# facebookresearch/vggsfm

Hardware: AMD Instinct MI355X
Metric: BA LM-iterations/sec (higher is better)
Workload: dtype f64

## Files before the change

vggsfm_amd/ba.py:

```python
import copy
import ctypes
from dataclasses import dataclass
from typing import Optional

import math
import os

import numpy as np
import torch

from . import _lib
from .ba_options import LOSS_ID, TERMINATION, BundleAdjustmentOptions

MODEL_ID = {"SIMPLE_PINHOLE": 0, "SIMPLE_RADIAL": 1}
GROUP = 16
CHUNK = 1024
SUB = 32
MIN_CHUNK = 128
OVERLAP_FACTORIZATION = False
OVERLAP_MIN_OBS, OVERLAP_MIN_FRAMES = 1_000_000, 8 * GROUP
TILE_BATCHES = 3
CHOL_CUS = 32


# ... 629 lines not shown
    overlap = OVERLAP_FACTORIZATION if overlap is None else bool(overlap)
    nb = TILE_BATCHES if (overlap and int(obs_cam.shape[0]) >= OVERLAP_MIN_OBS and S >= OVERLAP_MIN_FRAMES) else 1
    merged = nb == 1 and int(obs_cam.shape[0]) < MERGED_TILE_MAX_OBS
    merged_slots = slots[0] if merged else None
    chunk_desc, entries, tile_desc, obs_slot, nseg, batch_desc = build_schur_tiles(
        row_ptr, obs_cam, max_chunks=slots, num_batches=nb, later_scale=(cus - CHOL_CUS) / cus,
        merged_slots=merged_slots, block_rows=block_rows, simple=int(obs_cam.shape[0]) < SIMPLE_WORKLIST_MAX_OBS, num_cams=S)
    prob = DeviceProblem(cam_q, cam_t, intr, pts, row_ptr, obs_cam, obs_uv, col_ptr, cobs_pt, cobs_uv, chunk_desc,
                         entries, tile_desc, obs_slot, nseg, MODEL_ID[camera_type], cam_const=cam_const,
                         batch_desc=batch_desc, chol_split=chol_split, cam_perm=cam_perm, merged_tile_launch=merged,
                         refine_focal=bool(refine_focal_length), refine_extra=bool(refine_extra_params))
    if first_group is not None:
        kd_max = 2 if camera_type == "SIMPLE_RADIAL" else 1
        prob.chol_first_blk = envelope_blocks(first_group, S, 6 * S + kd_max * n_intr).to(dev)
    return prob, valid_idx, deleted


def window_bundle_adjustment(points3d, extrinsics, intrinsics, tracks, masks, num_existing_points, extra_params=None,
                             shared_camera=True, camera_type="SIMPLE_RADIAL", options=None):
    options = copy.deepcopy(options) if options is not None else BundleAdjustmentOptions()
    options.refine_focal_length = False
    options.refine_extra_params = False
    valid = masks.bool().sum(0) >= 2
    order = torch.cumsum(valid.long(), 0) - 1
    constant = valid & (order < num_existing_points)
    return bundle_adjustment(points3d, extrinsics, intrinsics, tracks, masks, None, extra_params, shared_camera,
                             camera_type, options, False, constant_points=constant, constant_pose_frames=[0],
                             filter_negative_depth=False)


def _c_options(options: BundleAdjustmentOptions, overlap=True):
    so = options.solver_options
    return _lib.BAOptions(so.max_num_iterations, so.max_num_consecutive_invalid_steps, int(so.jacobi_scaling),
                          so.function_tolerance, so.gradient_tolerance, so.parameter_tolerance,
                          so.initial_trust_region_radius, so.max_trust_region_radius, so.min_trust_region_radius,
                          so.min_lm_diagonal, so.max_lm_diagonal, so.min_relative_decrease,
                          CHOL_CUS if (overlap and OVERLAP_FACTORIZATION) else 0)


def _summary_dict(summ, log, n):
    its = [dict(iteration=l.iteration, cost=l.cost, cost_change=l.cost_change, gradient_max_norm=l.gradient_max_norm,
                step_norm=l.step_norm, relative_decrease=l.relative_decrease, radius=l.radius,
                successful=bool(l.successful)) for l in log[:n]]
    return dict(initial_cost=summ.initial_cost, final_cost=summ.final_cost, num_iterations=summ.num_iterations,
                num_successful_steps=summ.num_successful_steps, num_unsuccessful_steps=summ.num_unsuccessful_steps,
                termination=summ.termination, termination_str=TERMINATION.get(summ.termination, "?"),
                n_reduced=summ.n_reduced, iterations=its)


def apply_launch_hooks(L):
    glue = _hook("VGGSFM_LEGACY_GLUE")
    if glue is not None:
        L.vgg_ba_set_tile_rhs(2 | (4 if glue == "1" else 0))


def solve(problem: DeviceProblem, options: Optional[BundleAdjustmentOptions] = None, workspace=None):
    L = _lib.lib()
    apply_launch_hooks(L)
    options = options or BundleAdjustmentOptions()
    problem.refine_focal = options.refine_focal_length
    problem.refine_extra = options.refine_extra_params
    problem.loss = LOSS_ID[options.loss_function_type]
    problem.loss_scale = options.loss_function_scale
    cp = problem.c_struct()
    co = _c_options(options)
    nbytes = L.vgg_ba_workspace_bytes(ctypes.byref(cp), ctypes.byref(co))
    if workspace is None or workspace.numel() < nbytes:
        workspace = torch.empty(nbytes, dtype=torch.uint8, device=problem.pts.device)
    summ = _lib.BASummary()
    cap = options.solver_options.max_num_iterations + 2
    log = (_lib.BAIteration * cap)()
    _lib.check(L.vgg_ba_solve(ctypes.byref(cp), ctypes.byref(co), workspace, workspace.numel(), ctypes.byref(summ), log, cap,
                              _lib.stream_ptr()), "vgg_ba_solve")
    out = _summary_dict(summ, log, summ.num_log)
    if options.print_summary:
        print(f"Bundle adjustment report: residuals {problem.num_obs * 2}, parameters reduced {summ.n_reduced}, "
              f"iterations {summ.num_iterations}, cost {summ.initial_cost:.6g} -> {summ.final_cost:.6g}, "
              f"{out['termination_str']}")
    return out, workspace


POSE_COMPONENTS = ("rx", "ry", "rz", "tx", "ty", "tz")


@dataclass
class BACovariance:
    pose: Optional[torch.Tensor]
    intrinsics: Optional[torch.Tensor]
    pose_intrinsics: Optional[torch.Tensor]
    points: Optional[torch.Tensor]
    reduced: Optional[torch.Tensor]
    columns: list
    num_active: int
    variance_factor: float
    cost: float


def covariance_columns(problem: DeviceProblem):
    C, NI = problem.cam_t.shape[0], problem.intr.shape[0]
    names = [nm for nm, on in (("f", problem.refine_focal), ("k", problem.refine_extra and problem.camera_model == 1)) if on]
    frame = list(range(C)) if problem.cam_perm is None else [int(f) for f in problem.cam_perm.tolist()]
    cols = [("pose", frame[c], comp) for c in range(C) for comp in POSE_COMPONENTS]
    cols += [("intrinsics", 0 if NI == 1 else frame[a], nm) for a in range(NI) for nm in names]
    return cols


# ... 175 lines not shown
```

vggsfm_amd/csrc/ba.hip:

```cpp
#include <mutex>
#include <vector>

#include "ba_types.hpp"

namespace vgg {

Tuning g_tuning = {0, -1, 0, 0, 2, 0};
Profiler g_prof;

__global__ void init_kernel(DevProblem pb, Ws w, vgg_ba_options opt, int rank, int world) {
  const Dims& d = pb.d;
  const int j = blockIdx.x * blockDim.x + threadIdx.x;
  if (j == 0) {
    Ctl c;
    memset(&c, 0, sizeof(c));
    c.radius = opt.initial_trust_region_radius; c.decrease_factor = 2.0; c.need_lin = 1; c.rank = rank; c.world = world;
    *w.ctl = c;
    w.gmax_pts[0] = 0; for (int i = 0; i < 4; ++i) w.stepsum[i] = 0;
  }
  if (j < d.n_red) {
    bool act;
    if (j < 6 * d.C) {
      const int c = j / 6, k = j - 6 * c;
      const unsigned f = pb.cam_const ? pb.cam_const[c] : 0u;
      act = (pb.col_ptr[c + 1] > pb.col_ptr[c]) || world > 1;
      if (f & 1u) act = false;
      if (k >= 3 && (f & (2u << (k - 3)))) act = false;
    } else {
      const int a = (j - 6 * d.C) / d.kd;
      act = !(pb.intr_const && pb.intr_const[a]);
      if (!d.shared && world == 1 && !(pb.col_ptr[a + 1] > pb.col_ptr[a])) act = false;
    }
    w.active[j] = act ? 1 : 0;
    w.scale_c[j] = 1.0;
  }
}

__device__ __forceinline__ void begin_iteration(const Ws& w, const vgg_ba_options& opt) {
  Ctl* c = w.ctl;
  if (c->need_lin) {
    c->gmax = fmax(c->gmax_cams, w.gmax_pts[0]);
    w.log[c->iteration].gradient_max_norm = c->gmax;
    if (c->iteration == 0) {
      vgg_ba_iteration z;
      z.iteration = 0; z.successful = 1; z.cost = c->x_cost; z.cost_change = 0; z.gradient_max_norm = c->gmax;
      z.step_norm = 0; z.relative_decrease = 0; z.radius = c->radius;
      w.log[0] = z;
    }
    if (c->gmax <= opt.gradient_tolerance) { c->done = 1; c->termination = 1; return; }
  }
  if (c->iteration >= opt.max_num_iterations) { c->done = 1; c->termination = 0; return; }
  if (c->radius <= opt.min_trust_region_radius) { c->done = 1; c->termination = 4; return; }
  c->scale_ready = 1;
  c->need_lin = 0;
  c->iteration += 1;
}


__global__ __launch_bounds__(256) void begin_iteration_kernel(Ws w, vgg_ba_options opt, int n, int32_t* chol_flags, int chol_flag_count) {
  if (w.ctl->done) return;
// ... 284 lines not shown
  switch (phase) {
    case 0: return VGG_OK;
    case 1: phase_schur(L); return VGG_OK;
    case 2: return phase_step(L);
    case 3: phase_update(L); return VGG_OK;
    case 4: case 5: case 6: launch_pack_lower(L, phase - 4); return VGG_OK;
    case 7: case 9: case 12:
      if (L.num_batches != 1 || L.merged_tile_launch || L.d.C <= kGroup) return VGG_ERR_UNSUPPORTED;
      if (phase == 12) {
        launch_split_offsets(L);
        return VGG_OK;
      }
      phase_schur(L, phase == 7 ? 1 : 2);
      return VGG_OK;
    case 8: case 10:
      launch_pack_split(L, phase == 8 ? 0 : 1, 0);
      return VGG_OK;
    case 11:
      launch_pack_split(L, 0, 2);
      launch_pack_split(L, 1, 2);
      return VGG_OK;
    default: return VGG_ERR_INVALID_ARGUMENT;
  }
}

static int finish(const Launch& L, int max_iters, vgg_ba_summary* summary, vgg_ba_iteration* log, int log_cap) {
  Ctl h;
  if (hipMemcpyAsync(&h, L.w.ctl, sizeof(Ctl), hipMemcpyDeviceToHost, L.st) != hipSuccess) return VGG_ERR_HIP;
  int ncopy = 0;
  if (log && log_cap > 0) {
    ncopy = (max_iters + 1 < log_cap) ? max_iters + 1 : log_cap;
    if (hipMemcpyAsync(log, L.w.log, sizeof(vgg_ba_iteration) * ncopy, hipMemcpyDeviceToHost, L.st) != hipSuccess) return VGG_ERR_HIP;
  }
  if (hipStreamSynchronize(L.st) != hipSuccess) return VGG_ERR_HIP;
  if (summary) {
    summary->initial_cost = h.initial_cost; summary->final_cost = h.x_cost;
    summary->num_iterations = h.iteration; summary->num_successful_steps = h.num_succ;
    summary->num_unsuccessful_steps = h.num_unsucc; summary->termination = h.termination;
    summary->n_reduced = L.d.n_red;
    summary->num_log = (h.iteration + 1 < ncopy) ? h.iteration + 1 : ncopy;
  }
  return VGG_OK;
}

}

using namespace vgg;

extern "C" {

int vgg_ba_tuning(int lanes_per_point, int long_tracks, int cam_workgroups, int point_workgroups) {
  if (!(lanes_per_point == 0 || lanes_per_point == 8 || lanes_per_point == 16 || lanes_per_point == 32 || lanes_per_point == 64))
    return VGG_ERR_INVALID_ARGUMENT;
  vgg::g_tuning = vgg::Tuning{lanes_per_point, long_tracks < 0 ? -1 : (long_tracks ? 1 : 0), cam_workgroups > 0 ? cam_workgroups : 0,
                              point_workgroups > 0 ? point_workgroups : 0, vgg::g_tuning.tile_rhs, vgg::g_tuning.legacy_glue};
  return VGG_OK;
}

int vgg_ba_set_tile_rhs(int enable) {
  const bool known = enable >= 0 && enable <= 7 && (enable & 3) <= 2;
  vgg::g_tuning.tile_rhs = known ? (enable & 3) : 1;
  vgg::g_tuning.legacy_glue = (known && (enable & 4)) ? 1 : 0;
  return VGG_OK;
}

int vgg_ba_profile(int enable, int max_launches_per_kernel) {
  for (int k = 0; k < kProfCount; ++k) {
    for (int i = 0; i < g_prof.cap; ++i) { (void)hipEventDestroy(g_prof.start[k][i]); (void)hipEventDestroy(g_prof.stop[k][i]); }
    delete[] g_prof.start[k]; delete[] g_prof.stop[k];
    g_prof.start[k] = g_prof.stop[k] = nullptr; g_prof.n[k] = 0;
  }
  g_prof.cap = 0; g_prof.on = false;
  if (!enable) return VGG_OK;
  if (max_launches_per_kernel <= 0) return VGG_ERR_INVALID_ARGUMENT;
  for (int k = 0; k < kProfCount; ++k) {
    g_prof.start[k] = new hipEvent_t[max_launches_per_kernel];
    g_prof.stop[k] = new hipEvent_t[max_launches_per_kernel];
    for (int i = 0; i < max_launches_per_kernel; ++i) {
      VGG_HIP_CHECK(hipEventCreate(&g_prof.start[k][i]));
      VGG_HIP_CHECK(hipEventCreate(&g_prof.stop[k][i]));
    }
  }
  g_prof.cap = max_launches_per_kernel; g_prof.on = true;
  return VGG_OK;
}

int vgg_ba_profile_read(int kernel_id, double* total_ms, int* launches, int reset) {
  if (kernel_id < 0 || kernel_id >= kProfCount || !total_ms || !launches) return VGG_ERR_INVALID_ARGUMENT;
  double tot = 0;
  for (int i = 0; i < g_prof.n[kernel_id]; ++i) {
    VGG_HIP_CHECK(hipEventSynchronize(g_prof.stop[kernel_id][i]));
    float ms = 0;
    VGG_HIP_CHECK(hipEventElapsedTime(&ms, g_prof.start[kernel_id][i], g_prof.stop[kernel_id][i]));
    tot += ms;
  }
  *total_ms = tot; *launches = g_prof.n[kernel_id];
  if (reset) g_prof.n[kernel_id] = 0;
  return VGG_OK;
}

const char* vgg_build_arch(void) { return "gfx950"; }
int vgg_abi_version(void) { return VGG_ABI_VERSION; }
size_t vgg_abi_sizeof(int which) {
  switch (which) {
    case 0: return sizeof(vgg_ba_problem);
    case 1: return sizeof(vgg_ba_options);
    case 2: return sizeof(vgg_ba_iteration);
    case 3: return sizeof(vgg_ba_summary);
// ... 103 lines not shown
```

vggsfm_amd/csrc/ba_obs.hpp:

```cpp
#pragma once
#include "ba_types.hpp"

namespace vgg {

template <int N>
struct ObsPf {
  static_assert(N == 2 || N == 4, "prefetch depth");
  int c0 = 0, c1 = 0, c2 = 0, c3 = 0, s0 = 0, s1 = 0, s2 = 0, s3 = 0;
  float2 u0 = make_float2(0.f, 0.f), u1 = make_float2(0.f, 0.f), u2 = make_float2(0.f, 0.f), u3 = make_float2(0.f, 0.f);
  template <bool SLOT>
  __device__ __forceinline__ void load(const int32_t* cam, const float2* uv, const int32_t* slot, int o0, int o1, int stride, int sl) {
    int o = o0 + sl;
    if (o < o1) { c0 = cam[o]; u0 = uv[o]; if (SLOT) s0 = slot[o]; }
    o += stride;
    if (o < o1) { c1 = cam[o]; u1 = uv[o]; if (SLOT) s1 = slot[o]; }
    if (N == 4) {
      o += stride;
      if (o < o1) { c2 = cam[o]; u2 = uv[o]; if (SLOT) s2 = slot[o]; }
      o += stride;
      if (o < o1) { c3 = cam[o]; u3 = uv[o]; if (SLOT) s3 = slot[o]; }
    }
  }
  template <typename T>
  __device__ __forceinline__ static T pick(T a0, T a1, T a2, T a3, int k) {
    const T lo = (k & 1) ? a1 : a0, hi = (k & 1) ? a3 : a2;
    return (N == 4 && (k & 2)) ? hi : lo;
  }
  __device__ __forceinline__ int cam(int k, const int32_t* src, int o) const { return k < N ? pick(c0, c1, c2, c3, k) : src[o]; }
  __device__ __forceinline__ int slot(int k, const int32_t* src, int o) const { return k < N ? pick(s0, s1, s2, s3, k) : src[o]; }
  __device__ __forceinline__ float2 uv(int k, const float2* src, int o) const {
    if (k >= N) return src[o];
    return make_float2(pick(u0.x, u1.x, u2.x, u3.x, k), pick(u0.y, u1.y, u2.y, u3.y, k));
  }
};

struct CamR {
  double R[9];
  __device__ __forceinline__ explicit CamR(const double* q) { quat_to_R(q, R); }
};

template <int KD>
__device__ __forceinline__ double eval_full(const Dims& d, const double* Rm, const double* t, const double* in4,
                                            const double* X, float2 uv, unsigned camflag, bool intr_c, bool pt_c,
                                            double* r, double* F, double* E, double* Jw = nullptr) {
  constexpr int BD = 6 + KD;
  double Jp[12], Ji[4];
  obs_eval_R(d.model, Rm, t, in4, X, (double)uv.x, (double)uv.y, r, Jp, Ji, E);
#pragma unroll
  for (int row = 0; row < 2; ++row) {
#pragma unroll
    for (int k = 0; k < 6; ++k) F[row * BD + k] = Jp[row * 6 + k];
    if (KD == 2) { F[row * BD + 6] = Ji[row * 2]; F[row * BD + 7] = Ji[row * 2 + 1]; }
    if (KD == 1) F[row * BD + 6] = d.only_k ? Ji[row * 2 + 1] : Ji[row * 2];
  }
  const double s = r[0] * r[0] + r[1] * r[1];
  double rho[3];
  loss_eval(d.loss, d.loss_scale, s, rho);
  if (d.loss != kLossTrivial) {
    Corrector c(s, rho);
    c.jac<BD>(r, F);
    c.jac<3>(r, E);
    r[0] *= c.residual_scaling; r[1] *= c.residual_scaling;
  }
  if (Jw) {
#pragma unroll
    for (int k = 0; k < 3; ++k) { Jw[k] = F[3 + k]; Jw[3 + k] = F[BD + 3 + k]; }
  }
  if (camflag) {
#pragma unroll
    for (int k = 0; k < 3; ++k) {
      if (camflag & 1u) { F[k] = 0; F[BD + k] = 0; }
      if ((camflag & 1u) || (camflag & (2u << k))) { F[3 + k] = 0; F[BD + 3 + k] = 0; }
    }
  }
  if (intr_c) {
#pragma unroll
    for (int k = 0; k < KD; ++k) { F[6 + k] = 0; F[BD + 6 + k] = 0; }
  }
  if (pt_c) {
#pragma unroll
    for (int k = 0; k < 6; ++k) E[k] = 0;
  }
  return rho[0];
}

__device__ __forceinline__ double loss_rho0(const Dims& d, double s) {
  double rho[3];
  loss_eval(d.loss, d.loss_scale, s, rho);
  return rho[0];
}

template <int NV>
// ... 56 lines not shown
```

vggsfm_amd/csrc/ba_point.hip:

```cpp
#include "ba_obs.hpp"

namespace vgg {

#ifndef VGG_PP_ABLATE
#define VGG_PP_ABLATE 0
#endif
#ifndef VGG_PP_OCC
#define VGG_PP_OCC 2
#endif
#ifndef VGG_PS_OCC
#define VGG_PS_OCC 2
#endif

template <int KD, bool LDSCAM, bool CY, int LPP, bool LONGT = false>
__global__ __launch_bounds__(256, VGG_PP_OCC) void point_pass_kernel(DevProblem pb, Ws w, vgg_ba_options opt) {
  constexpr int BD = 6 + KD;
  __shared__ double wmax[4];
  extern __shared__ double cam_cache[];
  Ctl* ctl = w.ctl;
  if (ctl->done) return;
  const Dims& d = pb.d;
  constexpr int PPW = 64 / LPP;
  const int wave = threadIdx.x >> 6, lane = threadIdx.x & 63;
  const int sub = lane / LPP, sl = lane % LPP;
  const int nw = gridDim.x * 4 * PPW;
  const bool first = !ctl->scale_ready;
  const double radius = ctl->radius;
  const int kdsh = d.kdsh;
  double gmax = 0.0;
  const bool trhs = w.tile_rhs != 0;
  if (trhs) {
    zero_system_lower(w, pb.d.n_red, (int)blockIdx.x, (int)gridDim.x);
  }
  constexpr int KQ = (KD > 0) ? KD + KD * KD : 1;
  __shared__ double qs[4][64 / LPP][KQ];
  __shared__ __attribute__((aligned(16))) double2 ystage[CY ? 4 : 1][CY ? 64 * (kYc / 2) : 1];
  __shared__ int32_t slotstage[CY ? 4 : 1][CY ? 64 : 1];
  if (trhs && KD > 0 && (lane % LPP) == 0) {
#pragma unroll
    for (int i = 0; i < KQ; ++i) qs[wave][lane / LPP][i] = 0.0;
  }
  const double* lq = cam_cache;
  const double* lt = lq + 9 * d.C;
  const double* lsc = lt + 3 * d.C;
  const double* lfl = lsc + 6 * d.C;
  if (LDSCAM) {
    for (int i = threadIdx.x; i < d.C; i += 256) {
      quat_to_R(pb.cam_q + 4 * i, cam_cache + 9 * i);
      cam_cache[18 * d.C + i] = pb.cam_const ? (double)pb.cam_const[i] : 0.0;
    }
    for (int i = threadIdx.x; i < 3 * d.C; i += 256) cam_cache[9 * d.C + i] = pb.cam_t[i];
    for (int i = threadIdx.x; i < 6 * d.C; i += 256) cam_cache[12 * d.C + i] = w.scale_c[i];
    __syncthreads();
  }
  int p = (blockIdx.x * 4 + wave) * PPW + sub;
  constexpr int NPF = LONGT ? 4 : 2;
  constexpr bool CACHEJ = !LONGT;
  int n_o0 = 0, n_o1 = 0;
  ObsPf<NPF> n_pf;
  double n_X0 = 0, n_X1 = 0, n_X2 = 0;
  int n_ptc = 0;
  int m_o0 = 0, m_o1 = 0;
  double m_X0 = 0, m_X1 = 0, m_X2 = 0;
  int m_ptc = 0;
  if (p < d.P) {
    n_o0 = pb.row_ptr[p]; n_o1 = pb.row_ptr[p + 1];
    n_X0 = pb.pts[3 * p]; n_X1 = pb.pts[3 * p + 1]; n_X2 = pb.pts[3 * p + 2];
    n_ptc = pb.pt_const ? (int)pb.pt_const[p] : 0;
// ... 106 lines not shown
      const double l00 = sqrt(a00);
      const double l10 = a10 / l00, l20 = a20 / l00;
      const double d11 = a11 - l10 * l10;
      ok = ok && d11 > 0;
      const double l11 = sqrt(d11);
      const double l21 = (a21 - l20 * l10) / l11;
      const double d22 = a22 - l20 * l20 - l21 * l21;
      ok = ok && d22 > 0;
      const double l22 = sqrt(d22);
      if (!ok) { if (sl == 0) ctl->linear_fail = 1; }
      const double i00 = 1 / l00, i11 = 1 / l11, i22 = 1 / l22;
      const double i10 = -l10 * i00 * i11;
      const double i21 = -l21 * i11 * i22;
      const double i20 = -(l20 * i00 + l21 * i10) * i22;
      Gm[0] = s[0] * i00; Gm[1] = s[0] * i10; Gm[2] = s[0] * i20; Gm[3] = s[1] * i11; Gm[4] = s[1] * i21; Gm[5] = s[2] * i22;
      const double gs0 = s[0] * g[0], gs1 = s[1] * g[1], gs2 = s[2] * g[2];
      const double z0 = i00 * gs0, z1 = i10 * gs0 + i11 * gs1, z2 = i20 * gs0 + i21 * gs1 + i22 * gs2;
      hs[0] = Gm[0] * z0 + Gm[1] * z1 + Gm[2] * z2; hs[1] = Gm[3] * z1 + Gm[4] * z2; hs[2] = Gm[5] * z2;
      if (trhs && sl == 0) {
        double* Z = w.Zp + 9 * (size_t)p;
        Z[0] = z0; Z[1] = z1; Z[2] = z2;
        if (KD == 0) { Z[3] = 0; Z[4] = 0; Z[5] = 0; Z[6] = 0; Z[7] = 0; Z[8] = 0; }
        if (KD == 1 && kdsh) { Z[6] = 0; Z[7] = 0; Z[8] = 0; }
      }
      z_written = true;
      if (KD > 0 && kdsh) {
#pragma unroll
        for (int m = 0; m < KD; ++m) {
          const double sa = w.scale_c[6 * d.C + m];
          const double w0 = sa * s[0] * Wa[m * 3], w1 = sa * s[1] * Wa[m * 3 + 1], w2 = sa * s[2] * Wa[m * 3 + 2];
          const double y0 = i00 * w0, y1 = i10 * w0 + i11 * w1, y2 = i20 * w0 + i21 * w1 + i22 * w2;
          Ms[m * 3] = Gm[0] * y0 + Gm[1] * y1 + Gm[2] * y2; Ms[m * 3 + 1] = Gm[3] * y1 + Gm[4] * y2; Ms[m * 3 + 2] = Gm[5] * y2;
          if (trhs && sl == 0) { double* Z = w.Zp + 9 * (size_t)p + 3 + 3 * m; Z[0] = y0; Z[1] = y1; Z[2] = y2; }
        }
        if (trhs && sl == 0) {
          double* q = qs[wave][sub];
#pragma unroll
          for (int i = 0; i < KD; ++i) {
            q[i] += Wa[i * 3] * hs[0] + Wa[i * 3 + 1] * hs[1] + Wa[i * 3 + 2] * hs[2];
#pragma unroll
            for (int j = 0; j < KD; ++j)
              q[KD + i * KD + j] += Wa[i * 3] * Ms[j * 3] + Wa[i * 3 + 1] * Ms[j * 3 + 1] + Wa[i * 3 + 2] * Ms[j * 3 + 2];
          }
        }
      }
      gmax = fmax(gmax, fmax(fabs(g[0]), fmax(fabs(g[1]), fabs(g[2]))));
    }
    if (VGG_PP_ABLATE != 2) {
      const int bdt = d.shared ? 6 : BD;
      auto emit = [&](const int pass, const int o, const double* keptJ) __attribute__((always_inline)) {
        const bool head = pass == 0;
        const int c = f_pf.cam(pass, pb.obs_cam, o);
        double F[CY ? 6 : 2 * BD], E[6];
        if (KEEPJ && keptJ) {
          double Rl[9];
          const double* Rc = Rl;
          if (LDSCAM) Rc = lq + 9 * c; else quat_to_R(pb.cam_q + 4 * c, Rl);
#pragma unroll
          for (int i = 0; i < 6; ++i) F[i] = keptJ[i];
#pragma unroll
          for (int row = 0; row < 2; ++row)
#pragma unroll
            for (int k = 0; k < 3; ++k)
              E[3 * row + k] = pt_c ? 0.0 : keptJ[3 * row] * Rc[k] + keptJ[3 * row + 1] * Rc[3 + k] + keptJ[3 * row + 2] * Rc[6 + k];
        } else if (CACHEJ && !KEEPJ && head) {
#pragma unroll
          for (int i = 0; i < (CY ? 6 : 2 * BD); ++i) F[i] = cF[i];
#pragma unroll
          for (int i = 0; i < 6; ++i) E[i] = cE[i];
        } else {
          const int a = d.shared ? 0 : c;
          double r[2], Ff[2 * BD];
          const float2 uv = f_pf.uv(pass, pb.obs_uv, o);
          if (LDSCAM)
            eval_full<KD>(d, lq + 9 * c, lt + 3 * c, pb.intr + 4 * a, X, uv, (unsigned)lfl[c],
                          pb.intr_const ? pb.intr_const[a] != 0 : false, pt_c, r, CY ? Ff : F, E, CY ? F : nullptr);
          else
            eval_full<KD>(d, CamR(pb.cam_q + 4 * c).R, pb.cam_t + 3 * c, pb.intr + 4 * a, X, uv,
                          pb.cam_const ? pb.cam_const[c] : 0u, pb.intr_const ? pb.intr_const[a] != 0 : false, pt_c, r,
                          CY ? Ff : F, E, CY ? F : nullptr);
        }
        const int slot = f_pf.slot(pass, pb.obs_slot, o);
        if constexpr (CY) {
          double M[6];
          M[0] = E[0] * Gm[0]; M[1] = E[0] * Gm[1] + E[1] * Gm[3]; M[2] = E[0] * Gm[2] + E[1] * Gm[4] + E[2] * Gm[5];
          M[3] = E[3] * Gm[0]; M[4] = E[3] * Gm[1] + E[4] * Gm[3]; M[5] = E[3] * Gm[2] + E[4] * Gm[4] + E[5] * Gm[5];
          double rec[kYc];
#pragma unroll
          for (int i = 0; i < 3; ++i)
#pragma unroll
            for (int m = 0; m < 3; ++m) rec[3 * i + m] = F[i] * M[m] + F[3 + i] * M[3 + m];
          double Rl[9];
          const double* Rc = Rl;
          if (LDSCAM) Rc = lq + 9 * c; else quat_to_R(pb.cam_q + 4 * c, Rl);
#pragma unroll
          for (int i = 0; i < 3; ++i) {
            const double ai = Rc[3 * i] * X[0] + Rc[3 * i + 1] * X[1] + Rc[3 * i + 2] * X[2];
            rec[9 + i] = ai + ai;
          }
          slotstage[wave][lane] = slot;
#pragma unroll
          for (int i = 0; i < kYc / 2; ++i) ystage[wave][lane * (kYc / 2) + i] = make_double2(rec[2 * i], rec[2 * i + 1]);
        } else {
        const int rt = kGroup * bdt;
        double* y = w.Y + (size_t)(slot >> 4) * (3 * rt) + (slot & 15) * bdt;
        const bool pairs = (bdt & 1) == 0;
        double prev[3] = {0, 0, 0};
#pragma unroll
        for (int i = 0; i < BD; ++i) {
          if (i < bdt) {
            const double sc = (i < 6) ? (LDSCAM ? lsc[6 * c + i] : w.scale_c[6 * c + i])
                                      : w.scale_c[6 * d.C + KD * c + (i - 6)];
            const double w0 = F[i] * E[0] + F[BD + i] * E[3], w1 = F[i] * E[1] + F[BD + i] * E[4],
                         w2 = F[i] * E[2] + F[BD + i] * E[5];
            const double y0 = sc * (w0 * Gm[0]), y1 = sc * (w0 * Gm[1] + w1 * Gm[3]), y2 = sc * (w0 * Gm[2] + w1 * Gm[4] + w2 * Gm[5]);
#if VGG_PP_ABLATE == 1
            if (Gm[0] == 12345.678) {
#endif
            if (!pairs) { y[i] = y0; y[rt + i] = y1; y[2 * rt + i] = y2; }
            else if (i & 1) {
              *reinterpret_cast<double2*>(y + i - 1) = make_double2(prev[0], y0);
              *reinterpret_cast<double2*>(y + rt + i - 1) = make_double2(prev[1], y1);
              *reinterpret_cast<double2*>(y + 2 * rt + i - 1) = make_double2(prev[2], y2);
            } else { prev[0] = y0; prev[1] = y1; prev[2] = y2; }
#if VGG_PP_ABLATE == 1
            }
#endif
          }
        }
        }
      };
      if constexpr (KEEPJ) {
        auto flush_records = [&]() __attribute__((always_inline)) {
#if VGG_PP_ABLATE != 1
#pragma unroll
          for (int k = 0; k < kYc / 2; ++k) {
            const int q = k * 64 + lane;
            const int r = (q * 10923) >> 16;
            const int pc = q - 6 * r;
            const int sdst = slotstage[wave][r];
            const double2 v = ystage[wave][q];
            if (sdst >= 0) reinterpret_cast<double2*>(w.Y)[(size_t)sdst * (kYc / 2) + pc] = v;
          }
#endif
        };
#pragma unroll
        for (int ps = 0; ps < NPF; ++ps) {
          const int o = o0 + sl + ps * LPP;
          if (!__any(o < o1)) break;
          if (o < o1) emit(ps, o, cJ[ps]); else slotstage[wave][lane] = -1;
          flush_records();
        }
        for (int pass = NPF; __any(o0 + sl + pass * LPP < o1); ++pass) {
          const int o = o0 + sl + pass * LPP;
          if (o < o1) emit(pass, o, nullptr); else slotstage[wave][lane] = -1;
          flush_records();
        }
      } else {
        for (int o = o0 + sl; o < o1; o += LPP) emit((o - o0) / LPP, o, nullptr);
      }
    }
    if (sl == 0 && pvalid) {
      if (first) { w.scale_p[3 * p] = s[0]; w.scale_p[3 * p + 1] = s[1]; w.scale_p[3 * p + 2] = s[2]; }
#pragma unroll
      for (int i = 0; i < 6; ++i) w.G[6 * (size_t)p + i] = Gm[i];
#pragma unroll
      for (int i = 0; i < 3; ++i) { w.hs[3 * (size_t)p + i] = hs[i]; w.pdamp[3 * (size_t)p + i] = pd[i]; }
      if (KD > 0 && kdsh) {
#pragma unroll
        for (int i = 0; i < 3 * KD; ++i) w.Ms[(size_t)p * 3 * kdsh + i] = Ms[i];
      }
      if (trhs && !z_written) {
#pragma unroll
        for (int i = 0; i < 9; ++i) w.Zp[9 * (size_t)p + i] = 0.0;
      }
    }
  }
  gmax = wave_max(gmax);
  if (lane == 0) wmax[wave] = gmax;
  __syncthreads();
  if (threadIdx.x == 0) w.part_B[blockIdx.x] = fmax(fmax(wmax[0], wmax[1]), fmax(wmax[2], wmax[3]));
  if (trhs && KD > 0) {
    __syncthreads();
    if (threadIdx.x < KQ) {
      double v = 0.0;
      for (int wv = 0; wv < 4; ++wv)
        for (int sb = 0; sb < 64 / LPP; ++sb) v += qs[wv][sb][threadIdx.x];
      w.part_Q[8 * blockIdx.x + threadIdx.x] = v;
    }
  }
}

template <int KD>
__device__ __forceinline__ void cam_update_body(const DevProblem& pb, const Ws& w, int c) {
  constexpr int BD = 6 + KD;
  const Dims& d = pb.d;
  double step = 0, xn = 0, mcc = 0;
  if (c < d.C) {
    double dl[6], dyc[BD];
#pragma unroll
    for (int k = 0; k < 6; ++k) {
      const int j = 6 * c + k;
      const double dyv = w.active[j] ? w.scale_c[j] * w.rhs[j] : 0.0;
      w.dy[j] = dyv;
      dyc[k] = dyv;
      dl[k] = -dyv;
    }
    double qn[4];
    quat_plus_select(pb.cam_q + 4 * c, dl, qn);
// ... 155 lines not shown
          const double rty = cor.alpha_sq_norm * (s.r[0] * y[0] + s.r[1] * y[1]);
          y[0] = cor.sqrt_rho1 * (y[0] - s.r[0] * rty);
          y[1] = cor.sqrt_rho1 * (y[1] - s.r[1] * rty);
        }
      }
      double v3[3];
      s.adjoint(y, v3);
      if (!pt_c) {
#pragma unroll
        for (int k = 0; k < 3; ++k) t3[k] += Rc[k] * v3[0] + Rc[3 + k] * v3[1] + Rc[6 + k] * v3[2];
      }
    };
    for (int o = o0 + sl; o < o1; o += LPP) evaluated((o - o0) / LPP, o);
#pragma unroll
    for (int i = 0; i < 3; ++i) t3[i] = group_sum<LPP>(t3[i]);
    const double u0 = G00 * t3[0], u1 = G01 * t3[0] + G11 * t3[1], u2 = G02 * t3[0] + G12 * t3[1] + G22 * t3[2];
    double ys[3];
    ys[0] = hs0 - (G00 * u0 + G01 * u1 + G02 * u2);
    ys[1] = hs1 - (G11 * u1 + G12 * u2);
    ys[2] = hs2 - (G22 * u2);
    if (sl == 0) {
      w.cand_pts[3 * (size_t)p] = X[0] - ys[0]; w.cand_pts[3 * (size_t)p + 1] = X[1] - ys[1]; w.cand_pts[3 * (size_t)p + 2] = X[2] - ys[2];
      s_step += ys[0] * ys[0] + ys[1] * ys[1] + ys[2] * ys[2];
      if (!pt_c) s_xn += X[0] * X[0] + X[1] * X[1] + X[2] * X[2];
      if (G22 != 0.0) {
        const double z2 = ys[2] / G22, z1 = (ys[1] - G12 * z2) / G11, z0 = (ys[0] - G01 * z1 - G02 * z2) / G00;
        s_mcc += 0.5 * (z0 * z0 + z1 * z1 + z2 * z2) + 0.5 * (pd0 * ys[0] * ys[0] + pd1 * ys[1] * ys[1] + pd2 * ys[2] * ys[2]);
      }
    }
  }
  s_mcc = wave_sum(s_mcc); s_step = wave_sum(s_step); s_xn = wave_sum(s_xn);
  if (lane == 0) { red[wave][0] = s_mcc; red[wave][1] = s_step; red[wave][2] = s_xn; }
  __syncthreads();
  if (threadIdx.x < 3) w.part_F[4 * blockIdx.x + 1 + threadIdx.x] = red[0][threadIdx.x] + red[1][threadIdx.x] + red[2][threadIdx.x] + red[3][threadIdx.x];
}

__global__ __launch_bounds__(256) void reduce_step_kernel(Ws w, int nparts, int C) {
  __shared__ double red[4][256];
  if (w.ctl->done) return;
  reduce_step_body<false>(w, nparts, C, red);
}

void launch_point_pass(const Launch& L) {
  ProfScope ps(kProfPointPass, L.st);
  const Dims& d = L.d;
  const size_t cam_lds = sizeof(double) * 19 * (size_t)d.C;
  dispatch_kd(d.kd, [&](auto kd) {
    constexpr int KD = decltype(kd)::value;
    auto launch_cy = [&](auto lpp, auto cy) {
      constexpr int LPP = decltype(lpp)::value;
      constexpr bool CY = decltype(cy)::value;
      const bool longt = long_tracks(LPP, L.d.P, L.d.O);
      const size_t cam_cap = (CY ? 53 : 64) * 1024;
      if (longt && LPP <= 32) {
        if (cam_lds <= cam_cap) point_pass_kernel<KD, true, CY, LPP, (LPP <= 32)><<<L.wgB, 256, cam_lds, L.st>>>(L.dp, L.w, L.opt);
        else point_pass_kernel<KD, false, CY, LPP, (LPP <= 32)><<<L.wgB, 256, 0, L.st>>>(L.dp, L.w, L.opt);
      } else if (cam_lds <= cam_cap) point_pass_kernel<KD, true, CY, LPP><<<L.wgB, 256, cam_lds, L.st>>>(L.dp, L.w, L.opt);
      else point_pass_kernel<KD, false, CY, LPP><<<L.wgB, 256, 0, L.st>>>(L.dp, L.w, L.opt);
    };
    auto launch = [&](auto lpp) {
      if constexpr (KD == 0) launch_cy(lpp, std::true_type{});
      else if (d.shared) launch_cy(lpp, std::true_type{});
      else launch_cy(lpp, std::false_type{});
    };
    dispatch_lpp(L.lpp, launch);
  });
}

void launch_point_step(const Launch& L) {
  const Dims& d = L.d;
  const size_t cam_lds = sizeof(double) * (12 * (size_t)d.C + (size_t)d.n_red);
  const bool lds_cam = cam_lds <= 64 * 1024;
  const int fused = (lds_cam && !g_tuning.legacy_glue) ? 1 : 0;
  dispatch_kd(d.kd, [&](auto kd) {
    constexpr int KD = decltype(kd)::value;
    if (!fused) cam_update_kernel<KD><<<div_up(d.C + 1, 64), 64, 0, L.st>>>(L.dp, L.w);
    ProfScope ps(kProfPointStep, L.st);
    dispatch_lpp(L.lpp, [&](auto lpp) {
      constexpr int LPP = decltype(lpp)::value;
      const bool longt = long_tracks(LPP, L.d.P, L.d.O);
      if (longt && LPP <= 32) {
        if (lds_cam) point_step_kernel<KD, true, LPP, (LPP <= 32)><<<L.wgB, 256, cam_lds, L.st>>>(L.dp, L.w, fused);
        else point_step_kernel<KD, false, LPP, (LPP <= 32)><<<L.wgB, 256, 0, L.st>>>(L.dp, L.w, 0);
      } else if (lds_cam) point_step_kernel<KD, true, LPP><<<L.wgB, 256, cam_lds, L.st>>>(L.dp, L.w, fused);
      else point_step_kernel<KD, false, LPP><<<L.wgB, 256, 0, L.st>>>(L.dp, L.w, 0);
    });
  });
}

void launch_reduce_step(const Launch& L) { reduce_step_kernel<<<1, 256, 0, L.st>>>(L.w, L.wgB, L.d.C); }

}
```

vggsfm_amd/csrc/ba_types.hpp:

```cpp
#pragma once
#include <type_traits>

#include "camera_model.hpp"
#include "../../include/vggsfm_amd.h"

namespace vgg {

int cholesky_solve_enqueue(double* A, double* b, int n, double* inv_blocks, int32_t* device_fail, const int32_t* skip_flag,
                           hipStream_t st, const CholOverlap* overlap, int split_a, int split_b, const int32_t* first_blk,
                           bool flags_cleared);
int32_t* cholesky_dataflow_flags(double* ws, int n, size_t* count);
size_t cholesky_workspace_bytes(int n);
void dataflow_signal(int32_t* flag, hipStream_t st);

constexpr int kGroup = 16;
constexpr int kSub = 32;
constexpr int kMaxWG = 2048;
constexpr int kCamSplitMax = 16;
constexpr int kCamNV = 48;
constexpr int kPackPad = 1024;

struct Ctl {
  double radius, decrease_factor, x_cost, initial_cost, gmax_cams, gmax, cand_cost, mcc, step_norm, rel;
  int32_t iteration, done, termination, need_lin, scale_ready, invalid_streak, num_succ, num_unsucc;
// ... 16 lines not shown
  vgg_ba_iteration* log;
  double *cand_q, *cand_t, *cand_intr, *cand_pts;
  double *scale_c, *scale_p, *colsq_c, *dsq_c, *dy;
  uint8_t* active;
  double* lin;
  double *U, *g, *costc;
  double* sys;
  double *S, *rhs;
  double* S2;
  double* gmax_pts;
  double* stepsum;
  double *G, *hs, *Ms;
  double *pdamp;
  double* T;
  double* part_B;
  double* part_F;
  double* packed;
  size_t packed_count;
  double* pk_mine;
  double* pk_gathered;
  double* cam_part;
  double* cam_split;
  double* Y;
  size_t y_bytes;
  double* chol_inv;
  double* tile_part;
  int32_t* batch_flags;
  double *Zp, *rz_part, *part_Q;
  unsigned long long* split_off;
  double* rz;
  int tile_rhs;
  double* lin_cand;
  double *U_cand, *g_cand, *cost_cand;
  size_t lin_count, sys_count, total_bytes;
};

inline size_t align_up(size_t x, size_t a) { return (x + a - 1) / a * a; }


inline Dims make_dims(const vgg_ba_problem* pb) {
  Dims d;
  d.C = pb->num_cams; d.P = pb->num_pts; d.O = pb->num_obs; d.NI = pb->num_intr; d.model = pb->camera_model;
  const int rf = pb->refine_focal ? 1 : 0, rk = (pb->refine_extra && pb->camera_model == kSimpleRadial) ? 1 : 0;
  d.kd = rf + rk;
  d.only_k = (!rf && rk) ? 1 : 0;
  d.shared = (pb->num_intr == 1) ? 1 : 0;
  d.BDp = 6 + d.kd;
  d.n_red = 6 * d.C + d.kd * d.NI;
  d.kdsh = d.shared ? d.kd : 0;
  d.loss = pb->loss; d.loss_scale = pb->loss_scale;
  return d;
}

struct Tuning { int lpp, longt, cam_wgs, point_wgs, tile_rhs, legacy_glue; };
extern Tuning g_tuning;

inline Ws carve(const Dims& d, int max_iters, int num_chunks, int num_segments, void* base) {
  Ws w;
  size_t off = 0;
  auto take = [&](size_t bytes) { size_t o = off; off = align_up(off + bytes, 256); return (char*)base + o; };
  w.ctl = (Ctl*)take(sizeof(Ctl));
  w.log = (vgg_ba_iteration*)take(sizeof(vgg_ba_iteration) * (size_t)(max_iters + 2));
  w.cand_q = (double*)take(8ull * 4 * d.C); w.cand_t = (double*)take(8ull * 3 * d.C);
  w.cand_intr = (double*)take(8ull * 4 * d.NI); w.cand_pts = (double*)take(8ull * 3 * d.P);
  w.scale_c = (double*)take(8ull * d.n_red); w.scale_p = (double*)take(8ull * 3 * d.P);
  w.colsq_c = (double*)take(8ull * d.n_red); w.dsq_c = (double*)take(8ull * d.n_red);
  w.dy = (double*)take(8ull * d.n_red);
  w.active = (uint8_t*)take(d.n_red);
  w.lin_count = (size_t)d.C * d.BDp * d.BDp + (size_t)d.C * d.BDp + d.C;
  w.lin = (double*)take(8ull * w.lin_count);
  w.U = w.lin; w.g = w.U + (size_t)d.C * d.BDp * d.BDp; w.costc = w.g + (size_t)d.C * d.BDp;
  w.sys_count = (size_t)d.n_red * d.n_red + d.n_red;
  w.sys = (double*)take(8ull * w.sys_count);
  w.S = w.sys; w.rhs = w.S + (size_t)d.n_red * d.n_red;
  w.S2 = (double*)take(8ull * (size_t)d.n_red * d.n_red);
  w.packed_count = (size_t)d.n_red * (d.n_red + 1) / 2 + d.n_red;
  w.packed = (double*)take(8ull * (w.packed_count + 2 * kPackPad));
  w.pk_mine = (double*)take(8ull * (w.packed_count + 2));
  w.pk_gathered = (double*)take(8ull * (w.packed_count + 3 * kPackPad));
  w.gmax_pts = (double*)take(64);
  w.stepsum = (double*)take(64);
  w.G = (double*)take(8ull * 6 * d.P); w.hs = (double*)take(8ull * 3 * d.P);
  w.pdamp = (double*)take(8ull * 3 * d.P);
  w.Ms = (double*)take(8ull * 3 * (d.kdsh ? d.kdsh : 1) * d.P);
  w.T = (double*)take(8ull * d.C * d.BDp * (1 + d.kdsh));
  w.part_B = (double*)take(8ull * kMaxWG);
  w.part_F = (double*)take(8ull * kMaxWG * 4);
  w.cam_part = (double*)take(8ull * (d.C + 1) * 3);
  w.cam_split = (double*)take(8ull * (size_t)d.C * kCamSplitMax * kCamNV);
  w.y_bytes = 8ull * ((size_t)(num_segments > 0 ? num_segments : 0) + 1) * kGroup * y_slot_doubles(d);
  w.Y = (double*)take(w.y_bytes);
  w.chol_inv = (double*)take(cholesky_workspace_bytes(d.n_red));
  {
    const size_t bdt = d.shared ? 6 : d.BDp;
    w.tile_part = (double*)take(8ull * (size_t)(num_chunks > 0 ? num_chunks : 1) * bdt * bdt * 256);
  }
  w.batch_flags = (int32_t*)take(64);
  w.Zp = (double*)take(8ull * 9 * (d.P > 0 ? d.P : 1));
  w.rz_part = (double*)take(8ull * (size_t)(num_chunks > 0 ? num_chunks : 1) * kGroup * 6 * 3);
  w.part_Q = (double*)take(8ull * kMaxWG * 8);
  w.rz = (double*)take(8ull * (size_t)((d.C + kGroup - 1) / kGroup) * kGroup * 6 * 3);
  w.split_off = (unsigned long long*)take(8ull * 2 * ((size_t)d.n_red + 2));
  w.lin_cand = (double*)take(8ull * w.lin_count);
  w.U_cand = w.lin_cand; w.g_cand = w.U_cand + (size_t)d.C * d.BDp * d.BDp; w.cost_cand = w.g_cand + (size_t)d.C * d.BDp;
  w.tile_rhs = 0;
  w.total_bytes = off;
  return w;
// ... 103 lines not shown
```

Measured before the change: 737.8.

## Use 32-bit byte offsets and batched stores for Y record flush in point pass

The point pass kernel now precomputes byte offsets for the Y slot at record time, turning each scatter store into a 32-bit add whenever the Y buffer fits in 4 GiB. The flush loop first loads all six 16-byte pieces, then stores them, and skips the per-lane slot check when every lane in the wave is full. The rotation matrix is now loaded into registers once and reused to compute the a2 term, so the keep-J path does not rebuild it a second time. An environment hook can force the old 64-bit addressing, and the new code path relies on the 32-bit offset arithmetic never overflowing.

```diff
diff --git a/vggsfm_amd/ba.py b/vggsfm_amd/ba.py
--- a/vggsfm_amd/ba.py
+++ b/vggsfm_amd/ba.py
@@ -705,6 +705,9 @@
     glue = _hook("VGGSFM_LEGACY_GLUE")
     if glue is not None:
         L.vgg_ba_set_tile_rhs(2 | (4 if glue == "1" else 0))
+    wide = _hook("VGGSFM_Y_ADDR64")
+    if wide is not None:
+        L.vgg_ba_tuning(0, -2 if wide == "1" else -1, 0, 0)
 
 
 def solve(problem: DeviceProblem, options: Optional[BundleAdjustmentOptions] = None, workspace=None):
diff --git a/vggsfm_amd/csrc/ba.hip b/vggsfm_amd/csrc/ba.hip
--- a/vggsfm_amd/csrc/ba.hip
+++ b/vggsfm_amd/csrc/ba.hip
@@ -5,7 +5,7 @@
 
 namespace vgg {
 
-Tuning g_tuning = {0, -1, 0, 0, 2, 0};
+Tuning g_tuning = {0, -1, 0, 0, 2, 0, 0};
 Profiler g_prof;
 
 __global__ void init_kernel(DevProblem pb, Ws w, vgg_ba_options opt, int rank, int world) {
@@ -396,8 +396,11 @@
 int vgg_ba_tuning(int lanes_per_point, int long_tracks, int cam_workgroups, int point_workgroups) {
   if (!(lanes_per_point == 0 || lanes_per_point == 8 || lanes_per_point == 16 || lanes_per_point == 32 || lanes_per_point == 64))
     return VGG_ERR_INVALID_ARGUMENT;
+  const bool wide = long_tracks <= -2 && long_tracks >= -4;
+  if (wide) long_tracks = -long_tracks - 3;
   vgg::g_tuning = vgg::Tuning{lanes_per_point, long_tracks < 0 ? -1 : (long_tracks ? 1 : 0), cam_workgroups > 0 ? cam_workgroups : 0,
-                              point_workgroups > 0 ? point_workgroups : 0, vgg::g_tuning.tile_rhs, vgg::g_tuning.legacy_glue};
+                              point_workgroups > 0 ? point_workgroups : 0, vgg::g_tuning.tile_rhs, vgg::g_tuning.legacy_glue,
+                              wide ? 1 : 0};
   return VGG_OK;
 }
 
diff --git a/vggsfm_amd/csrc/ba_obs.hpp b/vggsfm_amd/csrc/ba_obs.hpp
--- a/vggsfm_amd/csrc/ba_obs.hpp
+++ b/vggsfm_amd/csrc/ba_obs.hpp
@@ -38,6 +38,8 @@
   double R[9];
   __device__ __forceinline__ explicit CamR(const double* q) { quat_to_R(q, R); }
 };
+
+__device__ __forceinline__ void keep_branch() { asm volatile(""); }
 
 template <int KD>
 __device__ __forceinline__ double eval_full(const Dims& d, const double* Rm, const double* t, const double* in4,
diff --git a/vggsfm_amd/csrc/ba_point.hip b/vggsfm_amd/csrc/ba_point.hip
--- a/vggsfm_amd/csrc/ba_point.hip
+++ b/vggsfm_amd/csrc/ba_point.hip
@@ -13,7 +13,7 @@
 #endif
 
 template <int KD, bool LDSCAM, bool CY, int LPP, bool LONGT = false>
-__global__ __launch_bounds__(256, VGG_PP_OCC) void point_pass_kernel(DevProblem pb, Ws w, vgg_ba_options opt) {
+__global__ __launch_bounds__(256, VGG_PP_OCC) void point_pass_kernel(DevProblem pb, Ws w, vgg_ba_options opt, int y32) {
   constexpr int BD = 6 + KD;
   __shared__ double wmax[4];
   extern __shared__ double cam_cache[];
@@ -226,17 +226,33 @@
         const bool head = pass == 0;
         const int c = f_pf.cam(pass, pb.obs_cam, o);
         double F[CY ? 6 : 2 * BD], E[6];
+        double a2[3] = {0, 0, 0};
+        bool a_done = false;
         if (KEEPJ && keptJ) {
           double Rl[9];
           const double* Rc = Rl;
           if (LDSCAM) Rc = lq + 9 * c; else quat_to_R(pb.cam_q + 4 * c, Rl);
+          double Rr[9];
+#pragma unroll
+          for (int i = 0; i < 9; ++i) Rr[i] = Rc[i];
 #pragma unroll
           for (int i = 0; i < 6; ++i) F[i] = keptJ[i];
 #pragma unroll
           for (int row = 0; row < 2; ++row)
 #pragma unroll
             for (int k = 0; k < 3; ++k)
-              E[3 * row + k] = pt_c ? 0.0 : keptJ[3 * row] * Rc[k] + keptJ[3 * row + 1] * Rc[3 + k] + keptJ[3 * row + 2] * Rc[6 + k];
+              E[3 * row + k] = keptJ[3 * row] * Rr[k] + keptJ[3 * row + 1] * Rr[3 + k] + keptJ[3 * row + 2] * Rr[6 + k];
+          if (__any(pt_c)) {
+            keep_branch();
+#pragma unroll
+            for (int i = 0; i < 6; ++i) E[i] = pt_c ? 0.0 : E[i];
+          }
+#pragma unroll
+          for (int i = 0; i < 3; ++i) {
+            const double ai = Rr[3 * i] * X[0] + Rr[3 * i + 1] * X[1] + Rr[3 * i + 2] * X[2];
+            a2[i] = ai + ai;
+          }
+          a_done = true;
         } else if (CACHEJ && !KEEPJ && head) {
 #pragma unroll
           for (int i = 0; i < (CY ? 6 : 2 * BD); ++i) F[i] = cF[i];
@@ -264,15 +280,19 @@
           for (int i = 0; i < 3; ++i)
 #pragma unroll
             for (int m = 0; m < 3; ++m) rec[3 * i + m] = F[i] * M[m] + F[3 + i] * M[3 + m];
-          double Rl[9];
-          const double* Rc = Rl;
-          if (LDSCAM) Rc = lq + 9 * c; else quat_to_R(pb.cam_q + 4 * c, Rl);
-#pragma unroll
-          for (int i = 0; i < 3; ++i) {
-            const double ai = Rc[3 * i] * X[0] + Rc[3 * i + 1] * X[1] + Rc[3 * i + 2] * X[2];
-            rec[9 + i] = ai + ai;
-          }
-          slotstage[wave][lane] = slot;
+          if (!a_done) {
+            double Rl[9];
+            const double* Rc = Rl;
+            if (LDSCAM) Rc = lq + 9 * c; else quat_to_R(pb.cam_q + 4 * c, Rl);
+#pragma unroll
+            for (int i = 0; i < 3; ++i) {
+              const double ai = Rc[3 * i] * X[0] + Rc[3 * i + 1] * X[1] + Rc[3 * i + 2] * X[2];
+              a2[i] = ai + ai;
+            }
+          }
+#pragma unroll
+          for (int i = 0; i < 3; ++i) rec[9 + i] = a2[i];
+          slotstage[wave][lane] = slot < 0 ? -1 : (y32 ? (int32_t)((uint32_t)slot * (uint32_t)(kYc * 8)) : slot);
 #pragma unroll
           for (int i = 0; i < kYc / 2; ++i) ystage[wave][lane * (kYc / 2) + i] = make_double2(rec[2 * i], rec[2 * i + 1]);
         } else {
@@ -305,16 +325,37 @@
         }
       };
       if constexpr (KEEPJ) {
-        auto flush_records = [&]() __attribute__((always_inline)) {
+        static_assert(kYc == 12, "six 16-byte pieces per record");
+        auto flush_records = [&](const bool full) __attribute__((always_inline)) {
 #if VGG_PP_ABLATE != 1
-#pragma unroll
-          for (int k = 0; k < kYc / 2; ++k) {
+          typedef double dbl2 __attribute__((ext_vector_type(2)));
+          int sd[6], pc[3];
+          dbl2 v[6];
+#pragma unroll
+          for (int k = 0; k < 3; ++k) {
             const int q = k * 64 + lane;
             const int r = (q * 10923) >> 16;
-            const int pc = q - 6 * r;
-            const int sdst = slotstage[wave][r];
-            const double2 v = ystage[wave][q];
-            if (sdst >= 0) reinterpret_cast<double2*>(w.Y)[(size_t)sdst * (kYc / 2) + pc] = v;
+            pc[k] = q - 6 * r;
+            sd[k] = slotstage[wave][r];
+            sd[k + 3] = slotstage[wave][r + 32];
+          }
+#pragma unroll
+          for (int k = 0; k < 6; ++k) v[k] = reinterpret_cast<const dbl2*>(ystage[wave])[k * 64 + lane];
+          if (!full) {
+#pragma unroll
+            for (int k = 0; k < 6; ++k) asm volatile("" ::"v"(v[k]));
+          }
+          if (y32) {
+            char* const Yb = reinterpret_cast<char*>(w.Y);
+#pragma unroll
+            for (int k = 0; k < 6; ++k) {
+              const uint32_t off = (uint32_t)sd[k] + (uint32_t)(16 * pc[k % 3]);
+              if (full || sd[k] != -1) *reinterpret_cast<dbl2*>(Yb + (size_t)off) = v[k];
+            }
+          } else {
+#pragma unroll
+            for (int k = 0; k < 6; ++k)
+              if (sd[k] != -1) reinterpret_cast<dbl2*>(w.Y)[(size_t)sd[k] * (kYc / 2) + pc[k % 3]] = v[k];
           }
 #endif
         };
@@ -322,13 +363,14 @@
         for (int ps = 0; ps < NPF; ++ps) {
           const int o = o0 + sl + ps * LPP;
           if (!__any(o < o1)) break;
+          const bool full = __all(o < o1 && f_pf.slot(ps, pb.obs_slot, o) >= 0);
           if (o < o1) emit(ps, o, cJ[ps]); else slotstage[wave][lane] = -1;
-          flush_records();
+          if (full) flush_records(true); else flush_records(false);
         }
         for (int pass = NPF; __any(o0 + sl + pass * LPP < o1); ++pass) {
           const int o = o0 + sl + pass * LPP;
           if (o < o1) emit(pass, o, nullptr); else slotstage[wave][lane] = -1;
-          flush_records();
+          flush_records(false);
         }
       } else {
         for (int o = o0 + sl; o < o1; o += LPP) emit((o - o0) / LPP, o, nullptr);
@@ -590,11 +632,12 @@
       constexpr bool CY = decltype(cy)::value;
       const bool longt = long_tracks(LPP, L.d.P, L.d.O);
       const size_t cam_cap = (CY ? 53 : 64) * 1024;
+      const int y32 = (CY && L.w.y_bytes <= 0xFFFFFFFFull && !g_tuning.y_addr64) ? 1 : 0;
       if (longt && LPP <= 32) {
-        if (cam_lds <= cam_cap) point_pass_kernel<KD, true, CY, LPP, (LPP <= 32)><<<L.wgB, 256, cam_lds, L.st>>>(L.dp, L.w, L.opt);
-        else point_pass_kernel<KD, false, CY, LPP, (LPP <= 32)><<<L.wgB, 256, 0, L.st>>>(L.dp, L.w, L.opt);
-      } else if (cam_lds <= cam_cap) point_pass_kernel<KD, true, CY, LPP><<<L.wgB, 256, cam_lds, L.st>>>(L.dp, L.w, L.opt);
-      else point_pass_kernel<KD, false, CY, LPP><<<L.wgB, 256, 0, L.st>>>(L.dp, L.w, L.opt);
+        if (cam_lds <= cam_cap) point_pass_kernel<KD, true, CY, LPP, (LPP <= 32)><<<L.wgB, 256, cam_lds, L.st>>>(L.dp, L.w, L.opt, y32);
+        else point_pass_kernel<KD, false, CY, LPP, (LPP <= 32)><<<L.wgB, 256, 0, L.st>>>(L.dp, L.w, L.opt, y32);
+      } else if (cam_lds <= cam_cap) point_pass_kernel<KD, true, CY, LPP><<<L.wgB, 256, cam_lds, L.st>>>(L.dp, L.w, L.opt, y32);
+      else point_pass_kernel<KD, false, CY, LPP><<<L.wgB, 256, 0, L.st>>>(L.dp, L.w, L.opt, y32);
     };
     auto launch = [&](auto lpp) {
       if constexpr (KD == 0) launch_cy(lpp, std::true_type{});
diff --git a/vggsfm_amd/csrc/ba_types.hpp b/vggsfm_amd/csrc/ba_types.hpp
--- a/vggsfm_amd/csrc/ba_types.hpp
+++ b/vggsfm_amd/csrc/ba_types.hpp
@@ -92,7 +92,7 @@
   return d;
 }
 
-struct Tuning { int lpp, longt, cam_wgs, point_wgs, tile_rhs, legacy_glue; };
+struct Tuning { int lpp, longt, cam_wgs, point_wgs, tile_rhs, legacy_glue, y_addr64; };
 extern Tuning g_tuning;
 
 inline Ws carve(const Dims& d, int max_iters, int num_chunks, int num_segments, void* base) {
```

Result: no change. 745.0, median of 6 (+1.0%).
